# burritojustice/reporter

Hardware: AMD Instinct MI355X
Metric: GPS points matched/sec (whole node) at 1/2/4/8 MI355X; % segment-ID agreement vs meili (higher is better)
Workload: dtype f32

## Files before the change

reporter_amd/csrc/kernels.hip:

```cpp
#include <hip/hip_runtime.h>

#include <algorithm>
#include <cstdlib>
#include <type_traits>

#include <hipcub/hipcub.hpp>

#include "kernels.h"
#include "otmatch.h"

namespace otm {

namespace {

#define MPD_F 111319.4954833f
constexpr uint32_t EMPTY = 0xFFFFFFFFu;
constexpr unsigned long long LAB_NONE = ~0ull;
constexpr int TB = 64;
__device__ __forceinline__ void wave_sync() {
  __builtin_amdgcn_wave_barrier();
  asm volatile("" ::: "memory");
}

__device__ __forceinline__ float cos_deg(float deg) {
// ... 1211 lines not shown

__device__ __forceinline__ uint32_t idx_hash(uint32_t v) {
  v ^= v >> 16;
  v *= 0x85ebca6bu;
  v ^= v >> 13;
  v *= 0xc2b2ae35u;
  v ^= v >> 16;
  return v;
}

constexpr int IDX_LOAD_FAST = 30, IDX_LOAD_DENSE = 40;
__host__ __device__ __forceinline__ int64_t idx_row_cap(int32_t c, int pct) {
  if (c <= 0) return 0;
  int64_t cap = ((int64_t)c * 100 + pct - 1) / pct;
  if (cap <= c) cap = (int64_t)c + 1;
  return (cap + 1) & ~(int64_t)1;
}
__device__ __forceinline__ uint32_t idx_slot0(uint32_t hh, const IdxRow& R) {
  return (uint32_t)(((uint64_t)hh * (uint64_t)(R.cap >> 1)) >> 32) << 1;
}
__device__ __forceinline__ uint32_t idx_next(uint32_t h, const IdxRow& R) {
  return h + 1u == R.cap ? 0u : h + 1u;
}
constexpr uint32_t IDX_LOW24 = 0xFFFFFFu;
constexpr uint32_t IDX_NO_PRED = 0xFFFFu;
static_assert((int64_t)INDEX_BUILD_LIMIT * 100 / IDX_LOAD_FAST + 2 < (int64_t)IDX_NO_PRED,
              "a row's slots must be numbered in 16 bits");
__host__ __device__ __forceinline__ uint32_t idx_slot_cost(const uint4& s) { return s.y & IDX_LOW24; }
__host__ __device__ __forceinline__ uint32_t idx_slot_units(const uint4& s) { return s.w & IDX_LOW24; }
__host__ __device__ __forceinline__ int32_t idx_slot_pred(const uint4& s) {
  const uint32_t p = (s.y >> 24) | ((s.w >> 24) << 8);
  return p == IDX_NO_PRED ? -1 : (int32_t)p;
}

__device__ __forceinline__ int64_t idx_find(const uint4* slot, const IdxRow& R, uint32_t v, uint4& out) {
  if (R.cnt < 0) return -2;
  if (R.cnt == 0) return -1;
  uint32_t h = idx_slot0(idx_hash(v), R);
  while (true) {
    const uint4 a = slot[R.off + h], b = slot[R.off + h + 1];
    if (a.x == v) {
      out = a;
      return R.off + h;
    }
    if (a.x == EMPTY) return -1;
    if (b.x == v) {
      out = b;
      return R.off + h + 1;
    }
    if (b.x == EMPTY) return -1;
    h = h + 2u == R.cap ? 0u : h + 2u;
  }
}
__device__ __forceinline__ int64_t src_row(const DevGraph& g, int32_t e, float off) {
  return cand_node(off) ? (int64_t)g.n_edges + g.e_from[e] : (int64_t)e;
}
__device__ __forceinline__ uint32_t dst_key(const DevGraph& g, int32_t e, float off) {
  return cand_node(off) ? NODE_KEY | (uint32_t)g.e_from[e] : (uint32_t)e;
}

template <bool WRITE>
__global__ __launch_bounds__(TB) void k_index_build(DevGraph g, const uint32_t* TU, uint32_t cmax, int32_t* row_cnt,
                                                    const IdxRow* rows, uint4* slot) {
  __shared__ uint32_t lkey[INDEX_BUILD_CAP];
  __shared__ unsigned long long llab[INDEX_BUILD_CAP];
  __shared__ uint32_t linq[INDEX_BUILD_CAP];
  __shared__ uint32_t lfr0[INDEX_BUILD_CAP];
  __shared__ uint32_t lfr1[INDEX_BUILD_CAP];
  __shared__ int32_t cbuf[CHAIN_BUF * TB];
  __shared__ SearchShared S;
  const int lane = threadIdx.x;
  const Table T{lkey, llab, linq, lfr0, lfr1, INDEX_BUILD_LOG2, INDEX_BUILD_LIMIT};
  const int64_t nrows = (int64_t)g.n_edges + g.n_nodes;
  for (int64_t r = blockIdx.x; r < nrows; r += gridDim.x) {
    const bool erow = r < g.n_edges;
    const int32_t u = erow ? g.e_to[r] : (int32_t)(r - g.n_edges);
    const uint32_t hin = erow ? (uint32_t)g.e_head_in[r] : NO_HEAD;
    const int n = ta_search<false>(g, TU, T, S, u, hin, cmax, lane);
    if (!WRITE) {
      if (lane == 0) row_cnt[r] = n;
      continue;
    }
    if (n < 0) continue;
    const IdxRow R = rows[r];
    auto predof = [&](uint32_t e) {
      const int sx = table_find<false>(T, e);
      return sx < 0 ? NONE_PRED : (uint32_t)(llab[sx] & 0xFFFFFFFFull);
    };
    for (int i = lane; i < INDEX_BUILD_CAP; i += TB) {
      const uint32_t k = lkey[i];
      if (k == EMPTY) continue;
      const unsigned long long lab = llab[i];
      const uint32_t pk = (uint32_t)(lab & 0xFFFFFFFFull);
      float d;
      uint32_t units;
      int len;
      chain_sums(g, TU, predof, pk, hin, (k & NODE_KEY) ? NO_HEAD : (uint32_t)g.e_head_out[k], cbuf + lane, d, units,
                 len);
      uint32_t h = idx_slot0(idx_hash(k), R);
      while (atomicCAS(&slot[R.off + h].x, EMPTY, k) != EMPTY) h = idx_next(h, R);
      slot[R.off + h].y = (uint32_t)(lab >> 32) & IDX_LOW24;
      slot[R.off + h].z = fbits(d);
      slot[R.off + h].w = units & IDX_LOW24;
    }
    __syncthreads();
    for (int i = lane; i < INDEX_BUILD_CAP; i += TB) {
      const uint32_t k = lkey[i];
      if (k == EMPTY) continue;
      const uint32_t pk = (uint32_t)(llab[i] & 0xFFFFFFFFull);
      uint4 sk_v, tmp;
      const int64_t sk = idx_find(slot, R, k, sk_v);
      const int64_t sp = pk == NONE_PRED ? -1 : idx_find(slot, R, pk, tmp);
      const uint32_t ps = sp < 0 ? IDX_NO_PRED : (uint32_t)(sp - R.off);
      slot[sk].y = (sk_v.y & IDX_LOW24) | (ps & 0xFFu) << 24;
      slot[sk].w = (sk_v.w & IDX_LOW24) | (ps >> 8) << 24;
    }
    __syncthreads();
  }
}

__global__ void k_row_sizes(const int32_t* row_cnt, int64_t* sizes, int32_t n, int pct) {
  const int32_t u = blockIdx.x * blockDim.x + threadIdx.x;
  if (u < n) sizes[u] = idx_row_cap(row_cnt[u], pct);
  if (u == n) sizes[n] = 0;
}

__global__ void k_row_pack(const int32_t* row_cnt, const int64_t* row_off, IdxRow* rows, int32_t n) {
  const int32_t u = blockIdx.x * blockDim.x + threadIdx.x;
  if (u >= n) return;
  const int64_t cap = row_off[u + 1] - row_off[u];
  rows[u] = IdxRow{row_off[u], row_cnt[u], (uint32_t)cap};
}

__global__ void k_src_pack(DevGraph g, const IdxRow* rows, SrcRec* src) {
  const int32_t e = blockIdx.x * blockDim.x + threadIdx.x;
  if (e >= g.n_edges) return;
  const int2 fl = g.e_fl[e];
  SrcRec r{};
  r.edge = rows[e];
  r.node = rows[(int64_t)g.n_edges + fl.x];
  r.from = fl.x;
  r.len = fl.y;
  src[e] = r;
}
__device__ __forceinline__ IdxRow src_row(const SrcRec* src, int32_t e, bool node) {
  const uint4 v = ((const uint4*)(src + e))[node ? 1 : 0];
  IdxRow R;
  R.off = (int64_t)((unsigned long long)v.x | (unsigned long long)v.y << 32);
  R.cnt = (int32_t)v.z;
  R.cap = v.w;
  return R;
}

#ifndef OTM_TRANS_KC8
#define OTM_TRANS_KC8 8
#endif
#ifndef OTM_TRANS_WAVES
#define OTM_TRANS_WAVES 8
#endif
template <int S, bool LIST>
__global__ __launch_bounds__(TB, OTM_TRANS_WAVES) void k_trans_sub(DevGraph g, DevBatch b, DevParams P, DevWork w) {
  if (*w.abort || trans_over_cap(b, w)) return;
  static_assert(S == 8 || S == 16, "8 lanes per column (two passes) or 16 (one pass / the wide pass)");
  constexpr int NS = TB / S;
  constexpr int KC = S >= 16 ? 16 : OTM_TRANS_KC8;
  constexpr bool WIDE = KC < 16;
  __shared__ int4 tg[NS][KC];
  __shared__ int4 sr[NS][KC];
  __shared__ IdxRow rq[NS][KC];
#ifndef OTM_TRANS_SWZ
#define OTM_TRANS_SWZ 1
#endif
  const int lane = threadIdx.x, sg = lane / S, sl = lane % S;
  const unsigned long long smask = ((1ull << S) - 1ull) << (sg * S);
  const int swz = !OTM_TRANS_SWZ ? 0 : (S == 8 ? ((sg >> 1) & 1) * 4 : (sg & 1) * 8);
  const DevIndex& X = w.idx;
  unsigned long long c_search = 0, c_settled = 0, c_relaxed = 0, c_trans = 0;
  const bool ordered = !LIST && (P.order_mask & ORDER_TRANS) != 0;
  int64_t base, end, stride;
  if (LIST) {
    base = (int64_t)blockIdx.x * NS;
    end = w.counters_i32[6];
    stride = (int64_t)gridDim.x * NS;
  } else if (ordered) {
    const int grp = blockIdx.x % ORDER_GROUPS;
    base = w.ord.grp[grp] + (int64_t)(blockIdx.x / ORDER_GROUPS) * NS;
    end = w.ord.grp[grp + 1];
    stride = (int64_t)(gridDim.x / ORDER_GROUPS) * NS;
  } else {
    base = (int64_t)blockIdx.x * NS;
    end = b.n_points;
    stride = (int64_t)gridDim.x * NS;
  }
  for (; base < end; base += stride) {
    const int64_t it = base + sg;
    bool act = it < end;
    int64_t p = 0;
    int32_t q = -1;
    int Kp = 0, Kq = 0;
    float gcv = 0.0f;
    int64_t toff = 0;
    if (act && ordered && w.colrec) {
      const int4 A = w.colrec[it];
      p = A.x;
      toff = w.trans_off[p];
      q = A.y;
      Kq = A.z & 255;
      Kp = A.z >> 8;
      gcv = __int_as_float(A.w);
    } else if (act) {
      p = LIST ? (int64_t)w.overflow_list2[it] : (ordered ? (int64_t)w.ord.item[it] : it);
      q = w.col_prev[p];
      Kq = w.kq_prev[p];
      Kp = w.ncand[p];
      gcv = w.gc[p];
      toff = w.trans_off[p];
    }
    act = act && q >= 0;
    const float bound = P.factor * gcv;
    const uint32_t cq = index_cost_bound(bound);
    const bool idx_ok = X.rmax > 0.0f && cq <= X.cmax;
#if OTM_SRC_REC
    const SrcRec* xsrc = X.src;
#else
    const IdxRow* xrow = X.row;
#endif
    const uint4* xslot = X.slot;
#pragma unroll
    for (int l = NEAR_LEVELS - 1; l >= 0; --l) {
      if (w.idxn[l].rmax > 0.0f && cq <= w.idxn[l].cmax) {
#if OTM_SRC_REC
        xsrc = w.idxn[l].src;
#else
        xrow = w.idxn[l].row;
#endif
        xslot = w.idxn[l].slot;
      }
    }
    const bool wide = WIDE && act && idx_ok && (Kp > KC || Kq > KC);
    if (wide && sl == 0) w.overflow_list2[atomicAdd(&w.counters_i32[6], 1)] = (int32_t)p;
    act = act && !wide;
    bool bad = act && (!idx_ok || Kp > KC || Kq > KC);
    for (int k = sl; k < KC; k += S) {
      if (act && k < Kp) {
        const int2 c = crec(w, p, k);
        const int32_t e = c.x;
        const float o = __int_as_float(c.y);
        const uint32_t key = dst_key(g, e, o);
        tg[sg][k ^ swz] = make_int4(e, __float_as_int(o), (int)key, (int)idx_hash(key));
      }
      if (act && k < Kq) {
        const int2 c = crec(w, q, k);
        const int32_t e = c.x;
        const float o = __int_as_float(c.y);
#if OTM_SRC_REC
        IdxRow R{};
        int32_t lenb;
        if (idx_ok) {
          R = src_row(xsrc, e, cand_node(o));
          lenb = xsrc[e].len;
        } else {
          lenb = g.e_fl[e].y;
        }
        const float start = cand_node(o) ? 0.0f : __int_as_float(lenb) - o;
        sr[sg][k ^ swz] = make_int4(e, __float_as_int(o), __float_as_int(start), w.ctr ? (int)src_head(g, e, o) : 0);
        if (idx_ok) {
          rq[sg][k ^ swz] = R;
          bad = bad || R.cnt < 0;
        }
#else
        const int2 fl = g.e_fl[e];
        const float start = cand_node(o) ? 0.0f : __int_as_float(fl.y) - o;
        sr[sg][k ^ swz] = make_int4(e, __float_as_int(o), __float_as_int(start), w.ctr ? (int)src_head(g, e, o) : 0);
        if (idx_ok) {
          const IdxRow R = xrow[cand_node(o) ? (int64_t)g.n_edges + fl.x : (int64_t)e];
          rq[sg][k ^ swz] = R;
          bad = bad || R.cnt < 0;
        }
#endif
      }
    }
    const bool spill = (__ballot(bad) & smask) != 0ull;
    if (spill && act && sl == 0) {
      const int slot = atomicAdd(&w.counters_i32[4], 1);
      w.overflow_list0[slot] = (int32_t)p;
    }
    act = act && !spill;
    wave_sync();
    if (act) {
      float* Tm = w.trans + toff;
      unsigned long long ntr = 0;
      constexpr int NB = OTM_TRANS_BATCH;
      const int npair = Kq * Kp;
      for (int idx0 = sl; idx0 < npair; idx0 += S * NB) {
        uint4 s0[NB], s1[NB];
        uint32_t h0[NB];
#pragma unroll
        for (int u = 0; u < NB; ++u) {
          const int idx = idx0 + u * S;
          s0[u] = make_uint4(EMPTY, 0u, 0u, 0u);
          s1[u] = s0[u];
          h0[u] = 0u;
          if (idx < npair) {
            const int i = idx / Kp, j = idx - (idx / Kp) * Kp;
            const int4 T = tg[sg][j ^ swz], Sx = sr[sg][i ^ swz];
            const IdxRow R = rq[sg][i ^ swz];
            const bool same = same_edge_step(Sx.x, __int_as_float(Sx.y), T.x, __int_as_float(T.y));
            if (!same && R.cnt > 0) {
              h0[u] = idx_slot0((uint32_t)T.w, R);
              s0[u] = xslot[R.off + h0[u]];
              s1[u] = xslot[R.off + h0[u] + 1];
            }
          }
        }
#pragma unroll
        for (int u = 0; u < NB; ++u) {
          const int idx = idx0 + u * S;
          if (idx >= npair) continue;
          const int i = idx / Kp, j = idx - (idx / Kp) * Kp;
          const int4 T = tg[sg][j ^ swz], Sx = sr[sg][i ^ swz];
          const uint32_t key = (uint32_t)T.z;
          const int32_t ej = T.x, ei = Sx.x;
          const float oj = __int_as_float(T.y), oi = __int_as_float(Sx.y), si = __int_as_float(Sx.z);
          float r = 0.0f;
          bool ok = true;
          uint32_t units = 0;
          if (same_edge_step(ei, oi, ej, oj)) {
            r = same_edge_dist(oi, oj);
          } else {
            const IdxRow R = rq[sg][i ^ swz];
            uint4 sv = s0[u];
            if (R.cnt > 0 && sv.x != key && sv.x != EMPTY) {
              sv = s1[u];
              uint32_t h = h0[u] + 1u;
              while (sv.x != key && sv.x != EMPTY) {
                h = idx_next(h, R);
                sv = xslot[R.off + h];
              }
            }
            if (R.cnt > 0 && sv.x == key && idx_slot_cost(sv) <= cq) {
              const float sd = si + bitsf(sv.z);
              r = sd + oj;
              units = idx_slot_units(sv);
            } else {
              ok = false;
            }
          }
          float cost = INFINITY;
          if (ok && r <= bound) {
            cost = trans_cost(units, r, gcv, P.beta);
            ++ntr;
          }
          Tm[i * Kp + j] = cost;
        }
      }
      if (w.ctr) {
        for (int i = 0; i < Kq; ++i) {
          const int4 Si = sr[sg][i ^ swz];
          const int32_t ui = src_node(g, Si.x, __int_as_float(Si.y));
          bool first = true;
          for (int k = 0; k < i; ++k) {
            const int4 Sk = sr[sg][k ^ swz];
            first = first && !(src_node(g, Sk.x, __int_as_float(Sk.y)) == ui && Sk.w == Si.w);
          }
          if (!first) continue;
          const IdxRow R = rq[sg][i ^ swz];
          for (int64_t k = sl; k < (int64_t)R.cap; k += S) {
            const uint4 slt = xslot[R.off + k];
            if (slt.x == EMPTY || (slt.x & NODE_KEY) || idx_slot_cost(slt) > cq) continue;
            ++c_settled;
            if ((unsigned long long)idx_slot_cost(slt) + g.e_len64[slt.x] <= cq) {
              const int32_t v = g.e_to[slt.x];
              c_relaxed += (unsigned long long)(g.out_off[v + 1] - g.out_off[v]);
            }
          }
          if (sl == 0) ++c_search;
        }
        c_trans += ntr;
      }
    }
    wave_sync();
  }
  if (w.ctr) {
    for (int sh = 32; sh > 0; sh >>= 1) {
      c_search += __shfl_xor(c_search, sh, 64);
      c_settled += __shfl_xor(c_settled, sh, 64);
      c_relaxed += __shfl_xor(c_relaxed, sh, 64);
      c_trans += __shfl_xor(c_trans, sh, 64);
    }
    if (lane == 0) {
      cadd(&w.ctr->searches, c_search);
      cadd(&w.ctr->nodes_settled, c_settled);
      cadd(&w.ctr->edges_relaxed, c_relaxed);
      cadd(&w.ctr->transitions, c_trans);
    }
  }
}

#ifndef OTM_ROUTE_WAVES
#define OTM_ROUTE_WAVES 1
#endif
__global__ __launch_bounds__(256, OTM_ROUTE_WAVES) void k_route_index(DevGraph g, DevBatch b, DevParams P, DevWork w) {
  if (*w.abort) return;
  const DevIndex& X = w.idx;
  unsigned long long c_search = 0, c_settled = 0, c_relaxed = 0, c_edges = 0;
  const ItemRange R = item_range(w, b, (P.order_mask & ORDER_ROUTE) != 0, 256);
  const bool rec = R.ordered && w.colrec && (P.order_mask & ORDER_TRANS);
  for (int64_t it = R.i0; it < R.i1; it += R.stride) {
    int64_t p;
    int32_t q = -1;
    float gcv = 0.0f;
    if (rec) {
      const int4 A = w.colrec[it];
      p = A.x;
      q = A.y;
      gcv = __int_as_float(A.w);
    } else {
      p = R.ordered ? (int64_t)w.ord.item[it] : it;
    }
    if (!R.ordered && !w.is_col[p]) continue;
    w.route_dist[p] = 0.0f;
    w.path_len[p] = 0;
    w.path_off[p] = 0;
    const int2 cq0 = w.chosen[q >= 0 ? q : p];
    if (w.state[p] < 0 || w.chain_start[p]) continue;
    if (!rec) {
      q = w.col_prev[p];
      gcv = w.gc[p];
    }
    const int2 ci = rec ? cq0 : w.chosen[q], cj = w.chosen[p];
    const int32_t ei = ci.x, ej = cj.x;
    const float oi = __int_as_float(ci.y), oj = __int_as_float(cj.y);
    if (same_edge_step(ei, oi, ej, oj)) {
      w.route_dist[p] = same_edge_dist(oi, oj);
      continue;
    }
    const float bound = P.factor * gcv;
    const uint32_t cq = index_cost_bound(bound);
    IdxRow Rw{};
    int64_t sv = -1;
    uint4 lab{};
    int lvl = -1;
#pragma unroll
    for (int l = NEAR_LEVELS - 1; l >= 0; --l)
      if (w.idxn[l].rmax > 0.0f && cq <= w.idxn[l].cmax) lvl = l;
    const DevIndex& Xc = lvl >= 0 ? w.idxn[lvl] : X;
#if OTM_SRC_REC
    int32_t leni = 0;
    if (X.rmax > 0.0f && cq <= X.cmax) {
      Rw = src_row(Xc.src, ei, cand_node(oi));
      leni = Xc.src[ei].len;
      sv = idx_find(Xc.slot, Rw, dst_key(g, ej, oj), lab);
    }
#else
    const int2 fli = g.e_fl[ei];
    const int32_t leni = fli.y;
    if (X.rmax > 0.0f && cq <= X.cmax) {
      Rw = Xc.row[cand_node(oi) ? (int64_t)g.n_edges + fli.x : (int64_t)ei];
      sv = idx_find(Xc.slot, Rw, dst_key(g, ej, oj), lab);
    }
#endif
    if (sv < 0 || idx_slot_cost(lab) > cq) {
      const int slot = atomicAdd(&w.counters_i32[4], 1);
      w.overflow_list0[slot] = (int32_t)p;
      continue;
    }
    int len = 0;
    for (int32_t ps = idx_slot_pred(lab); ps >= 0 && len <= Rw.cnt; ps = idx_slot_pred(Xc.slot[Rw.off + ps])) ++len;
    const int off = len ? atomicAdd(&w.counters_i32[1], len) : 0;
    if (off + len > w.pool_cap) {
      w.counters_i32[2] = 1;
      *w.abort = 1;
      w.path_len[p] = -1;
    } else {
      int k = len;
      for (int32_t ps = idx_slot_pred(lab); ps >= 0 && k > 0;) {
        const uint4 sl = Xc.slot[Rw.off + ps];
        w.path_pool[off + (--k)] = (int32_t)sl.x;
        ps = idx_slot_pred(sl);
      }
      w.path_off[p] = off;
      w.path_len[p] = len;
    }
    const float start = cand_node(oi) ? 0.0f : __int_as_float(leni) - oi;
    const float sd = start + bitsf(lab.z);
    w.route_dist[p] = sd + oj;
    if (w.ctr) {
      unsigned long long st = 0, rl = 0;
      for (int64_t k = 0; k < (int64_t)Rw.cap; ++k) {
        const uint4 sl = Xc.slot[Rw.off + k];
        if (sl.x == EMPTY || (sl.x & NODE_KEY) || idx_slot_cost(sl) > cq) continue;
        ++st;
        if ((unsigned long long)idx_slot_cost(sl) + g.e_len64[sl.x] <= cq) {
          const int32_t v = g.e_to[sl.x];
          rl += (unsigned long long)(g.out_off[v + 1] - g.out_off[v]);
        }
      }
      ++c_search;
      c_settled += st;
      c_relaxed += rl;
      c_edges += (unsigned long long)len;
    }
  }
  if (w.ctr) {
    cadd(&w.ctr->route_searches, c_search);
    cadd(&w.ctr->route_nodes_settled, c_settled);
    cadd(&w.ctr->route_edges_relaxed, c_relaxed);
    cadd(&w.ctr->route_edges, c_edges);
  }
}

template <int TIER>
__device__ __forceinline__ Table tier_table(const DevWork& w, uint32_t* lkey, unsigned long long* llab, uint32_t* linq,
                                            uint32_t* lfr0, uint32_t* lfr1) {
  if (TIER == 1) {
    const size_t base = (size_t)blockIdx.x * BIG_TABLE_CAP;
    return Table{w.big_key + base, w.big_lab + base, w.big_inq + base, w.big_fr + 2 * base,
                 w.big_fr + 2 * base + BIG_TABLE_CAP, BIG_TABLE_LOG2, SEARCH_LIMIT,
                 w.big_ins + (size_t)blockIdx.x * SEARCH_LIMIT, w.big_prev + blockIdx.x};
  }
  if (TIER == 2) {
    const size_t cap = (size_t)1 << w.huge_log2;
    const size_t base = (size_t)blockIdx.x * cap;
    const int lim = huge_limit(w.huge_log2);
    return Table{w.huge_key + base, w.huge_lab + base, w.huge_inq + base, w.huge_fr + 2 * base,
                 w.huge_fr + 2 * base + cap, w.huge_log2, lim, w.huge_ins + (size_t)blockIdx.x * lim,
                 w.huge_prev + blockIdx.x};
  }
  return Table{lkey, llab, linq, lfr0, lfr1, 8, LDS_TABLE_LIMIT};
}
__device__ __forceinline__ bool huge_unready(DevWork& w, int64_t nwork, const int32_t* list) {
  if (nwork <= 0 || w.huge_log2 > 0) return false;
  if (w.huge_final) {
// ... 2022 lines not shown
    const int pk = m - (has0 ? 1 : 0);
    if (has0 && m == 0) {
      pc = RoutePiece{ei, oi, g.e_len[ei], 0.0f};
    } else if (pk < plen) {
      const int32_t e = w.path_pool[poff + pk];
      const float len = g.e_len[e];
      pc = RoutePiece{e, 0.0f, len, start + dd};
      dd = dd + len;
    } else {
      pc = RoutePiece{ej, 0.0f, oj, start + dd};
    }
    const int32_t s0 = g.e_shape_off[pc.edge], nsh = g.e_shape_off[pc.edge + 1] - s0 - 1;
    float bsq = INFINITY, boff = 0.0f;
    for (int sg = 0; sg < nsh; ++sg) {
      float sqd, off;
      project(g, pc.edge, sg, lat, lon, ls, sqd, off);
      if (sqd < bsq) {
        bsq = sqd;
        boff = off;
      }
    }
    if (!(boff >= pc.o0 && boff <= pc.o1)) continue;
    const float pos = pc.xs + (boff - pc.o0);
    const float cost = bsq / ds + fabsf(pos - gcd) / P.beta;
    if (cost < best) {
      best = cost;
      bpos = pos;
    }
  }
  return bpos;
}

__global__ __launch_bounds__(256) void k_seg_bound(DevGraph g, DevBatch b, DevParams P, DevWork w, int64_t* tb) {
  const int64_t k = (int64_t)blockIdx.x * blockDim.x + threadIdx.x;
  if (OTM_FOLD_BOOKKEEPING && k == b.n_points) fold_snap(w, 2, false);
  if (*w.abort) return;
  const int lane = threadIdx.x & 63;
  int64_t v = 0;
  int32_t t = -1;
  if (k < b.n_points) {
    t = w.pt_trace[k];
    if (w.is_col[k]) {
      if (w.state[k] >= 0) {
        const int32_t pl = w.path_len[k];
        v = 2 + (pl > 0 ? pl : 0);
      }
    } else {
      const int32_t q = w.prevc[k];
      const int32_t p = q >= 0 ? w.nextc[q] : -1;
      if (p >= 0 && w.col_prev[p] == q && !w.chain_start[p] && w.state[p] >= 0 && w.path_len[p] >= 0 &&
          w.trace_err[t] == 0) {
        const int2 ci = w.chosen[q], cj = w.chosen[p];
        if (!same_edge_step(ci.x, __int_as_float(ci.y), cj.x, __int_as_float(cj.y)))
          w.ipos[k] = interp_pos(g, b, P, w, q, p, k);
      }
    }
  }
#pragma unroll
  for (int d = 1; d < 64; d <<= 1) {
    const int64_t vn = __shfl_down(v, d, 64);
    const int32_t tn = __shfl_down(t, d, 64);
    if (lane + d < 64 && tn == t) v += vn;
  }
  const int32_t tp = __shfl_up(t, 1, 64);
  if (t >= 0 && (lane == 0 || tp != t) && v != 0) atomicAdd((unsigned long long*)&tb[t], (unsigned long long)v);
}

__global__ __launch_bounds__(TB) void k_compact(int32_t n_traces, DevOut o, const int32_t* seg_off, const int32_t* way_off,
                                                const int32_t* rep_off, otm_segment* so, int64_t* wo,
                                                otm_report_rec* ro, otm_trace_result* to) {
  const int lane = threadIdx.x;
  const otm_trace_result* TR = (const otm_trace_result*)o.traces;
  const otm_segment* SI = (const otm_segment*)o.segments;
  const otm_report_rec* RI = (const otm_report_rec*)o.reports;
  for (int32_t t = blockIdx.x; t < n_traces; t += gridDim.x) {
    const int32_t base = TR[t].seg_off;
    const int32_t ns = o.seg_cnt[t], nw = o.way_cnt[t], nr = o.rep_cnt[t];
    const int32_t ds = seg_off[t], dw = way_off[t], dr = rep_off[t];
    for (int k = lane; k < ns; k += TB) {
      otm_segment x = SI[base + k];
      x.way_off = x.way_off - base + dw;
      so[ds + k] = x;
    }
    for (int k = lane; k < nw; k += TB) wo[dw + k] = o.way_ids[base + k];
    for (int k = lane; k < nr; k += TB) ro[dr + k] = RI[base + k];
    if (lane == 0) {
      otm_trace_result x = TR[t];
      x.seg_off = ds;
      x.rep_off = dr;
      to[t] = x;
    }
  }
}

__global__ __launch_bounds__(1024) void k_fetch_scan(int32_t n, const int32_t* c0, const int32_t* c1,
                                                     const int32_t* c2, int32_t* o0, int32_t* o1, int32_t* o2) {
  __shared__ int32_t ws[3][16];
  const int t = threadIdx.x, lane = t & 63, wv = t >> 6;
  int carry0 = 0, carry1 = 0, carry2 = 0;
  for (int base = 0; base < n; base += 1024) {
    const int i = base + t;
    const int s0 = i < n ? c0[i] : 0, s1 = i < n ? c1[i] : 0, s2 = i < n ? c2[i] : 0;
    int i0 = s0, i1 = s1, i2 = s2;
    for (int o = 1; o < 64; o <<= 1) {
      const int x0 = __shfl_up(i0, o, 64), x1 = __shfl_up(i1, o, 64), x2 = __shfl_up(i2, o, 64);
      if (lane >= o) {
        i0 += x0;
        i1 += x1;
        i2 += x2;
      }
    }
    if (lane == 63) {
      ws[0][wv] = i0;
      ws[1][wv] = i1;
      ws[2][wv] = i2;
    }
    __syncthreads();
    int b0 = 0, b1 = 0, b2 = 0, z0 = 0, z1 = 0, z2 = 0;
    for (int k = 0; k < 16; ++k) {
      const int w0 = ws[0][k], w1 = ws[1][k], w2 = ws[2][k];
      if (k < wv) {
        b0 += w0;
        b1 += w1;
        b2 += w2;
      }
      z0 += w0;
      z1 += w1;
      z2 += w2;
    }
    if (i < n) {
      o0[i] = carry0 + b0 + i0 - s0;
      o1[i] = carry1 + b1 + i1 - s1;
      o2[i] = carry2 + b2 + i2 - s2;
    }
    carry0 += z0;
    carry1 += z1;
    carry2 += z2;
    __syncthreads();
  }
  if (t == 0) {
    o0[n] = carry0;
    o1[n] = carry1;
    o2[n] = carry2;
  }
}

int grid_for(int64_t n, int per_block, int cap) {
  int64_t g = (n + per_block - 1) / per_block;
  if (g < 1) g = 1;
  return (int)(g > cap ? cap : g);
}

constexpr int WAVE_GRID_CAP = 256 * 64;
constexpr int TRANS_GRID_CAP = 65536;

}

void launch_fetch_scan(int32_t n, const int32_t* c0, const int32_t* c1, const int32_t* c2, int32_t* o0, int32_t* o1,
                       int32_t* o2, hipStream_t s) {
  hipLaunchKernelGGL(k_fetch_scan, dim3(1), dim3(1024), 0, s, n, c0, c1, c2, o0, o1, o2);
}


const char* const kKernelNames[KN_COUNT] = {
    "k_columns",       "spatial_order",  "k_cand_lane",    "k_candidates",     "k_links",         "scan_trans_off",  "k_trans_sub",
    "k_trans_wide",    "k_transitions",  "k_transitions_big", "k_viterbi",      "k_route_index",
    "k_route",         "k_route_big",    "k_seg_bound",      "scan_seg_bound",  "k_segments",       "k_report"};

namespace {
constexpr int SPILL_GRID = 4096;
#ifndef OTM_WIDE_GRID
#define OTM_WIDE_GRID 8192
#endif
constexpr int WIDE_GRID = OTM_WIDE_GRID;
}

#define TIMED(k, launch) \
  do {                   \
    mk.begin(k, s);      \
    launch;              \
    mk.end(k, s);        \
  } while (0)

void launch_columns(const DevGraph& g, const DevBatch& b, const DevParams& p, DevWork& w, hipStream_t s,
                    const Marks& mk) {
  if (w.ord.tile_cnt) (void)hipMemsetAsync(w.ord.tile_cnt, 0, ORDER_TILES * 4, s);
  TIMED(KN_COLUMNS, hipLaunchKernelGGL(k_columns, dim3(grid_for(b.n_traces, 1, WAVE_GRID_CAP)), dim3(TB), 0, s, g,
                                       b, p, w));
}
static int order_grid(int64_t n, int per_block, int cap) {
  const int64_t per_group = (n + ORDER_GROUPS - 1) / ORDER_GROUPS;
  int64_t gb = (per_group + per_group / 4 + per_block - 1) / per_block;
  if (gb < 1) gb = 1;
  int64_t gtot = gb * ORDER_GROUPS;
  if (gtot > cap) gtot = cap / ORDER_GROUPS * ORDER_GROUPS;
  return (int)gtot;
}

void launch_order(const DevBatch& b, DevWork& w, hipStream_t s, const Marks& mk) {
  mk.begin(KN_ORDER, s);
  hipLaunchKernelGGL(k_order_plan, dim3(1), dim3(1024), 0, s, w.ord.tile_cnt, w.ord.cursor, w.ord.grp);
  hipLaunchKernelGGL(k_order_scatter, dim3(grid_for(b.n_points, 256, 8192)), dim3(256), 0, s, b, w, w.ord.tile,
                     w.ord.cursor, w.ord.item);
  mk.end(KN_ORDER, s);
}

void launch_candidates(const DevGraph& g, const DevBatch& b, const DevParams& p, DevWork& w, hipStream_t s,
                       const Marks& mk, int from) {
  if (from < RESUME_CAND_BIG) {
    if (w.ctr)
      TIMED(KN_CAND_LANE, hipLaunchKernelGGL(k_cand_lane<true>, dim3(order_grid(b.n_points, CAND_TB, 1 << 30)),
                                             dim3(CAND_TB), 0, s, g, b, p, w));
    else
      TIMED(KN_CAND_LANE, hipLaunchKernelGGL(k_cand_lane<false>, dim3(order_grid(b.n_points, CAND_TB, 1 << 30)),
                                             dim3(CAND_TB), 0, s, g, b, p, w));
  }
  mk.begin(KN_CAND_WAVE, s);
  if (from < RESUME_CAND_BIG) hipLaunchKernelGGL(k_candidates<false>, dim3(4096), dim3(TB), 0, s, g, b, p, w);
  hipLaunchKernelGGL(k_candidates<true>, dim3(CAND_BIG_SLOTS), dim3(TB), 0, s, g, b, p, w);
  mk.end(KN_CAND_WAVE, s);
}
void launch_links(const DevBatch& b, const DevParams& p, DevWork& w, hipStream_t s, const Marks& mk) {
  TIMED(KN_LINKS, hipLaunchKernelGGL(k_links, dim3(grid_for(b.n_points + 1, 256, 1 << 30)), dim3(256), 0, s, b, p,
                                     w));
}
void launch_batch_init(int32_t* counters, int32_t* abort, hipStream_t s) {
  hipLaunchKernelGGL(k_batch_init, dim3(1), dim3(64), 0, s, counters, abort);
}
void launch_snap(int32_t* counters, int32_t* snap, bool reset, hipStream_t s) {
  hipLaunchKernelGGL(k_snap, dim3(1), dim3(64), 0, s, counters, snap, reset ? 1 : 0);
}
__global__ __launch_bounds__(256) void k_expand_compact(const int64_t* trace_off, const int64_t* tbase,
                                                        const int32_t* dt, const int16_t* acc16, double* time,
                                                        float* acc, int32_t n_traces) {
  const int wv = threadIdx.x >> 6, lane = threadIdx.x & 63;
  for (int64_t t = (int64_t)blockIdx.x * 4 + wv; t < n_traces; t += (int64_t)gridDim.x * 4) {
    const int64_t a = trace_off[t], e = trace_off[t + 1], base = tbase[t];
    for (int64_t i = a + lane; i < e; i += 64) {
      time[i] = (double)(base + (int64_t)dt[i]);
      acc[i] = (float)acc16[i];
    }
  }
}
void launch_expand_compact(const int64_t* trace_off, const int64_t* tbase, const int32_t* dt, const int16_t* acc16,
                           double* time, float* acc, int32_t n_traces, hipStream_t s) {
  if (n_traces <= 0) return;
  hipLaunchKernelGGL(k_expand_compact, dim3(grid_for(((int64_t)n_traces + 3) / 4, 1, 1 << 20)), dim3(256), 0, s,
                     trace_off, tbase, dt, acc16, time, acc, n_traces);
}
void launch_status(const int32_t* abort, const int64_t* ttotal, const int32_t* counters, BatchStatus* out,
                   hipStream_t s) {
  hipLaunchKernelGGL(k_status, dim3(1), dim3(64), 0, s, abort, ttotal, counters, out);
}
bool fold_bookkeeping() { return OTM_FOLD_BOOKKEEPING != 0; }
void launch_cap_check(const DevBatch& b, DevWork& w, hipStream_t s) {
  hipLaunchKernelGGL(k_cap_check, dim3(1), dim3(1), 0, s, b, w);
}
void launch_transitions(const DevGraph& g, const DevBatch& b, const DevParams& p, DevWork& w, hipStream_t s,
                        const Marks& mk, int sub, int from) {
  if (from >= RESUME_TRANS_HUGE) {
    mk.begin(KN_TRANS_GLOBAL, s);
    hipLaunchKernelGGL(k_transitions<2>, dim3(HUGE_SLOTS), dim3(TB), 0, s, g, b, p, w);
    mk.end(KN_TRANS_GLOBAL, s);
    return;
  }
  const int per = TB / sub;
  const int grid = order_grid((b.n_points + per - 1) / per, 1, TRANS_GRID_CAP);
  if (sub == 8) {
    TIMED(KN_TRANS_INDEX, hipLaunchKernelGGL((k_trans_sub<8, false>), dim3(grid), dim3(TB), 0, s, g, b, p, w));
    TIMED(KN_TRANS_WIDE, hipLaunchKernelGGL((k_trans_sub<16, true>), dim3(WIDE_GRID), dim3(TB), 0, s, g, b, p, w));
  } else {
    TIMED(KN_TRANS_INDEX, hipLaunchKernelGGL((k_trans_sub<16, false>), dim3(grid), dim3(TB), 0, s, g, b, p, w));
    mk.begin(KN_TRANS_WIDE, s);
    mk.end(KN_TRANS_WIDE, s);
  }
  TIMED(KN_TRANS_WAVE, hipLaunchKernelGGL(k_transitions<0>, dim3(SPILL_GRID), dim3(TB), 0, s, g, b, p, w));
  mk.begin(KN_TRANS_GLOBAL, s);
  hipLaunchKernelGGL(k_transitions<1>, dim3(BIG_SLOTS), dim3(TB), 0, s, g, b, p, w);
  hipLaunchKernelGGL(k_transitions<2>, dim3(HUGE_SLOTS), dim3(TB), 0, s, g, b, p, w);
  mk.end(KN_TRANS_GLOBAL, s);
}
void launch_viterbi(const DevBatch& b, DevWork& w, hipStream_t s, const Marks& mk) {
  const char* fe = std::getenv("OTM_VIT_FORM");
  const int forced = fe ? std::atoi(fe) : 0;
  constexpr int gmin = 32768;
  constexpr int rmin = 8192;
  const int form = forced ? forced : (b.n_traces >= gmin ? 8 : (b.n_traces >= rmin ? 4 : 64));
  if (form == 4) {
    const char* we = std::getenv("OTM_VR_WIN");
    const int vt = OTM_VR_U * 16;
    int win = we ? std::atoi(we) : vt;
    win = win < 0 ? 0 : (win > vt ? vt : win);
    mk.begin(KN_VITERBI, s);
    hipLaunchKernelGGL(k_viterbi_row, dim3(grid_for(b.n_traces, TB / 16, WAVE_GRID_CAP)), dim3(TB), 0, s, b, w,
                       w.overflow_list2, w.counters_i32 + 26, win, 1);
    hipLaunchKernelGGL(k_viterbi, dim3(grid_for(b.n_traces, 1, WAVE_GRID_CAP)), dim3(TB), 0, s, b, w,
                       (const int32_t*)w.overflow_list2, (const int32_t*)(w.counters_i32 + 26), 0);
    mk.end(KN_VITERBI, s);
    return;
  }
  if (form == 64) {
    TIMED(KN_VITERBI, hipLaunchKernelGGL(k_viterbi, dim3(grid_for(b.n_traces, 1, WAVE_GRID_CAP)), dim3(TB), 0, s, b,
                                         w, (const int32_t*)nullptr, (const int32_t*)nullptr, 1));
    return;
  }
  int32_t* l8 = w.overflow_list0;
  int32_t* n8 = w.counters_i32 + 20;
// ... 106 lines not shown
```

Baseline: 1.567 billion.

## Flatten transition pair loop across all subgroup columns in a wave

Instead of each S-lane subgroup iterating over its own column's Kq*Kp pairs, the wave computes prefix sums of pair counts across subgroups and lets all 64 lanes stride over the combined pair list. Per-column parameters (offset, gcv, bound, cq, slot pointer) are staged in shared memory so any lane can process any column's pair. This is meant to remove lane idling when columns have uneven pair counts, at the cost of a per-pair column lookup and extra LDS reads. The search-counting code is factored into a lambda, and the transition grid cap becomes a macro.

```diff
diff --git a/reporter_amd/csrc/kernels.hip b/reporter_amd/csrc/kernels.hip
--- a/reporter_amd/csrc/kernels.hip
+++ b/reporter_amd/csrc/kernels.hip
@@ -1387,8 +1387,18 @@
   return R;
 }
 
+__device__ __forceinline__ unsigned long long word64(int lo, int hi) {
+  return (unsigned long long)(uint32_t)lo | (unsigned long long)(uint32_t)hi << 32;
+}
+
 #ifndef OTM_TRANS_KC8
 #define OTM_TRANS_KC8 8
+#endif
+#ifndef OTM_TRANS_FLAT
+#define OTM_TRANS_FLAT 1
+#endif
+#if OTM_TRANS_FLAT && OTM_TRANS_BATCH != 1
+#error "the flat pair loop takes one pair per lane per step (OTM_TRANS_BATCH=1)"
 #endif
 #ifndef OTM_TRANS_WAVES
 #define OTM_TRANS_WAVES 8
@@ -1403,6 +1413,9 @@
   __shared__ int4 tg[NS][KC];
   __shared__ int4 sr[NS][KC];
   __shared__ IdxRow rq[NS][KC];
+#if OTM_TRANS_FLAT
+  __shared__ int4 cr[NS][2];
+#endif
 #ifndef OTM_TRANS_SWZ
 #define OTM_TRANS_SWZ 1
 #endif
@@ -1412,6 +1425,29 @@
   const DevIndex& X = w.idx;
   unsigned long long c_search = 0, c_settled = 0, c_relaxed = 0, c_trans = 0;
   const bool ordered = !LIST && (P.order_mask & ORDER_TRANS) != 0;
+  auto count_searches = [&](int Kq, uint32_t cq, const uint4* xslot) {
+    for (int i = 0; i < Kq; ++i) {
+      const int4 Si = sr[sg][i ^ swz];
+      const int32_t ui = src_node(g, Si.x, __int_as_float(Si.y));
+      bool first = true;
+      for (int k = 0; k < i; ++k) {
+        const int4 Sk = sr[sg][k ^ swz];
+        first = first && !(src_node(g, Sk.x, __int_as_float(Sk.y)) == ui && Sk.w == Si.w);
+      }
+      if (!first) continue;
+      const IdxRow R = rq[sg][i ^ swz];
+      for (int64_t k = sl; k < (int64_t)R.cap; k += S) {
+        const uint4 slt = xslot[R.off + k];
+        if (slt.x == EMPTY || (slt.x & NODE_KEY) || idx_slot_cost(slt) > cq) continue;
+        ++c_settled;
+        if ((unsigned long long)idx_slot_cost(slt) + g.e_len64[slt.x] <= cq) {
+          const int32_t v = g.e_to[slt.x];
+          c_relaxed += (unsigned long long)(g.out_off[v + 1] - g.out_off[v]);
+        }
+      }
+      if (sl == 0) ++c_search;
+    }
+  };
   int64_t base, end, stride;
   if (LIST) {
     base = (int64_t)blockIdx.x * NS;
@@ -1521,6 +1557,89 @@
       w.overflow_list0[slot] = (int32_t)p;
     }
     act = act && !spill;
+#if OTM_TRANS_FLAT
+    const int npair_g = act ? Kq * Kp : 0;
+    if (sl == 0) {
+      const unsigned long long xs = (unsigned long long)xslot;
+      cr[sg][0] = make_int4((int)(uint32_t)toff, (int)(uint32_t)((unsigned long long)toff >> 32),
+                            act ? (Kp | Kq << 8 | 1 << 16) : 0, __float_as_int(gcv));
+      cr[sg][1] = make_int4(__float_as_int(bound), (int)cq, (int)(uint32_t)xs, (int)(uint32_t)(xs >> 32));
+    }
+    wave_sync();
+    {
+      int pre[NS], total = 0;
+#pragma unroll
+      for (int c = 0; c < NS; ++c) {
+        pre[c] = total;
+        total += __builtin_amdgcn_readlane(npair_g, c * S);
+      }
+      unsigned long long ntr = 0;
+      for (int f = lane; f < total; f += TB) {
+        int c = 0, pc = 0;
+#pragma unroll
+        for (int k = 1; k < NS; ++k) {
+          if (f >= pre[k]) {
+            c = k;
+            pc = pre[k];
+          }
+        }
+        const int idx = f - pc;
+        const int cz = !OTM_TRANS_SWZ ? 0 : (S == 8 ? ((c >> 1) & 1) * 4 : (c & 1) * 8);
+        const int4 C0 = cr[c][0], C1 = cr[c][1];
+        const int kp = C0.z & 255;
+        const float gcv_c = __int_as_float(C0.w), bound_c = __int_as_float(C1.x);
+        const uint32_t cq_c = (uint32_t)C1.y;
+        const uint4* xslot_c = (const uint4*)word64(C1.z, C1.w);
+        const int64_t toff_c = (int64_t)word64(C0.x, C0.y);
+        const int i = idx / kp, j = idx - (idx / kp) * kp;
+        const int4 T = tg[c][j ^ cz], Sx = sr[c][i ^ cz];
+        const uint32_t key = (uint32_t)T.z;
+        const int32_t ej = T.x, ei = Sx.x;
+        const float oj = __int_as_float(T.y), oi = __int_as_float(Sx.y), si = __int_as_float(Sx.z);
+        float r = 0.0f;
+        bool ok = true;
+        uint32_t units = 0;
+        if (same_edge_step(ei, oi, ej, oj)) {
+          r = same_edge_dist(oi, oj);
+        } else {
+          const IdxRow R = rq[c][i ^ cz];
+          uint4 sv = make_uint4(EMPTY, 0u, 0u, 0u);
+          if (R.cnt > 0) {
+            uint32_t h = idx_slot0((uint32_t)T.w, R);
+            sv = xslot_c[R.off + h];
+            uint4 s1 = xslot_c[R.off + h + 1];
+            if (sv.x != key && sv.x != EMPTY) {
+              sv = s1;
+              h = h + 1u;
+              while (sv.x != key && sv.x != EMPTY) {
+                h = idx_next(h, R);
+                sv = xslot_c[R.off + h];
+              }
+            }
+          }
+          if (R.cnt > 0 && sv.x == key && idx_slot_cost(sv) <= cq_c) {
+            const float sd = si + bitsf(sv.z);
+            r = sd + oj;
+            units = idx_slot_units(sv);
+          } else {
+            ok = false;
+          }
+        }
+        float cost = INFINITY;
+        if (ok && r <= bound_c) {
+          cost = trans_cost(units, r, gcv_c, P.beta);
+          ++ntr;
+        }
+        w.trans[toff_c + idx] = cost;
+      }
+      if (w.ctr) {
+        const int4 C0 = cr[sg][0], C1 = cr[sg][1];
+        if (C0.z >> 16)
+          count_searches((C0.z >> 8) & 255, (uint32_t)C1.y, (const uint4*)word64(C1.z, C1.w));
+        c_trans += ntr;
+      }
+    }
+#else
     wave_sync();
     if (act) {
       float* Tm = w.trans + toff;
@@ -1590,30 +1709,11 @@
         }
       }
       if (w.ctr) {
-        for (int i = 0; i < Kq; ++i) {
-          const int4 Si = sr[sg][i ^ swz];
-          const int32_t ui = src_node(g, Si.x, __int_as_float(Si.y));
-          bool first = true;
-          for (int k = 0; k < i; ++k) {
-            const int4 Sk = sr[sg][k ^ swz];
-            first = first && !(src_node(g, Sk.x, __int_as_float(Sk.y)) == ui && Sk.w == Si.w);
-          }
-          if (!first) continue;
-          const IdxRow R = rq[sg][i ^ swz];
-          for (int64_t k = sl; k < (int64_t)R.cap; k += S) {
-            const uint4 slt = xslot[R.off + k];
-            if (slt.x == EMPTY || (slt.x & NODE_KEY) || idx_slot_cost(slt) > cq) continue;
-            ++c_settled;
-            if ((unsigned long long)idx_slot_cost(slt) + g.e_len64[slt.x] <= cq) {
-              const int32_t v = g.e_to[slt.x];
-              c_relaxed += (unsigned long long)(g.out_off[v + 1] - g.out_off[v]);
-            }
-          }
-          if (sl == 0) ++c_search;
-        }
+        count_searches(Kq, cq, xslot);
         c_trans += ntr;
       }
     }
+#endif
     wave_sync();
   }
   if (w.ctr) {
@@ -3942,7 +4042,10 @@
 }
 
 constexpr int WAVE_GRID_CAP = 256 * 64;
-constexpr int TRANS_GRID_CAP = 65536;
+#ifndef OTM_TRANS_GRID_CAP
+#define OTM_TRANS_GRID_CAP 65536
+#endif
+constexpr int TRANS_GRID_CAP = OTM_TRANS_GRID_CAP;
 
 }
 
```

Result: faster. 1.610 billion, median of 6 (+2.8%).
